# FARIDKH/Multi-agent-RL-for-FJSP

Hardware: AMD Instinct MI355X
Metric: env-steps/sec (all agents) at N parallel envs, 1/2/4/8 MI355X (higher is better)
Workload: dtype int32+f64; 1 GPU; fjsp_step_4096envs; envs_per_gpu=4096, global_envs=4096, num_orders=30, policy=random, steps_per_launch=1024, kernel=k_step_ag<lds,predraw>, bench_step=one rollout batch = 256 env-steps of each of the 4096 envs, env_steps_per_bench_step=1048576, parallelism=env-shard x1 (no data-path collective)

## Files before the change

### multi-agent-rl-for-fjsp_amd/csrc/fjsp_env.h

```cpp
#pragma once
#include <stdint.h>

#include "fjsp_stamps.h"

#ifndef FJSP_DEV
#define FJSP_DEV __device__ __forceinline__
#endif
#ifndef FJSP_HD
#ifdef __HIP__
#define FJSP_HD __host__ __device__ __forceinline__
#else
#define FJSP_HD FJSP_DEV
#endif
#endif

namespace fjsp {

FJSP_DEV float __uint_as_float_fjsp(uint32_t u) { float f; __builtin_memcpy(&f, &u, 4); return f; }
FJSP_DEV uint32_t __float_as_uint_fjsp(float f) { uint32_t u; __builtin_memcpy(&u, &f, 4); return u; }

constexpr int BLOCK = 64;
constexpr int NA = 8;
constexpr int NI32 = 20, NI8 = 12, NF32 = 6, NMASK = 29;
constexpr int MAX_ORDERS = 64;
// ... 637 lines not shown
    return inflight && cs == (uint16_t)step;
}
template <int S, bool AT = false>
FJSP_DEV void pack_run(Env& E, const Tables& T, const Cfg& C, int started, bool due, int* orders_done) {
    constexpr int L = L_PKG + S;
    const int step = E.step();
    const int qfirst = E.p_qfirst(S);
    if (started && E.p_inflight(S) + E.p_queued(S) > C.pkg_cap)
        E.flag(ST_PKG_WAIT | ST_DIVERGED);
    int done = 0;
    while (due) {
        const int s = list_pop<L>(E, T);
        const int code = T.scode[s * T.stride];
        const int o = tc_order(code);
        const uint32_t add = tc_range(code) << 9;
        uint32_t w = (AT ? order_or(&T.orders[o * T.stride], add) : T.orders[o * T.stride]) | add;
        const uint32_t full = (1u << ow_n(w)) - 1u;
        if (!(w & (1u << 18)) && ((w >> 9) & full) == full) {
            w |= 1u << 18;
            *orders_done += 1;
            if (AT) order_or(&T.orders[o * T.stride], 1u << 18);
        }
        if (!AT) T.orders[o * T.stride] = w;
        done += tc_count(code);
        due = E.ll(L) > 0 && E.lh(L) != qfirst && T.scstep[E.lh(L) * T.stride] == PKG_CONT;
    }
    if (done) {
        E.set_p_completed(S, E.p_completed(S) + done);
        E.set_total_packaged(E.total_packaged() + done);
        E.set_p_inflight(S, E.p_inflight(S) - done);
        E.set_p_busy(S, 0);
    }
    if (started) {
        T.scstep[qfirst * T.stride] = (uint16_t)(step + C.ptk_pack);
        const int inflight = E.p_inflight(S) + E.p_queued(S);
        E.w[20 + S] = 3u | ((uint32_t)NIL << 2) | ((uint32_t)(inflight & 0xFF) << 10);
    }
}

template <int S>
FJSP_DEV int pack_complete(Env& E, const Tables& T, bool due, int* orders_done) {
    constexpr int L = L_PKG + S;
    const int qfirst = E.p_qfirst(S);
    int done = 0;
    while (due) {
        const int s = list_pop<L>(E, T);
        const int code = T.scode[s * T.stride];
        const int o = tc_order(code);
        const uint32_t add = tc_range(code) << 9;
        const uint32_t w = order_or(&T.orders[o * T.stride], add) | add;
        const uint32_t full = (1u << ow_n(w)) - 1u;
        if (!(w & (1u << 18)) && ((w >> 9) & full) == full) {
            order_or(&T.orders[o * T.stride], 1u << 18);
            *orders_done += 1;
        }
        done += tc_count(code);
        due = E.ll(L) > 0 && E.lh(L) != qfirst && T.scstep[E.lh(L) * T.stride] == PKG_CONT;
    }
    return done;
}
template <int S>
FJSP_DEV void pack_finish(Env& E, const Tables& T, const Cfg& C, int started, int done) {
    if (started && E.p_inflight(S) + E.p_queued(S) > C.pkg_cap) E.flag(ST_PKG_WAIT | ST_DIVERGED);
    if (done) {
        E.set_p_completed(S, E.p_completed(S) + done);
        E.set_total_packaged(E.total_packaged() + done);
        E.set_p_inflight(S, E.p_inflight(S) - done);
        E.set_p_busy(S, 0);
    }
    if (started) {
        T.scstep[E.p_qfirst(S) * T.stride] = (uint16_t)(E.step() + C.ptk_pack);
        const int inflight = E.p_inflight(S) + E.p_queued(S);
        E.w[20 + S] = 3u | ((uint32_t)NIL << 2) | ((uint32_t)(inflight & 0xFF) << 10);
    }
}

template <int P>
struct PackSlot { static constexpr int value = P; };
template <int P, int NP, class F>
FJSP_DEV void pack_slots(F&& f) {
    if constexpr (P < NP) { f(PackSlot<P>{}); pack_slots<P + 1, NP>(f); }
}
template <int G>
FJSP_DEV uint32_t pack_lane_room(const Env& E, const Cfg& C, int g) {
    uint32_t room = 0;
#pragma unroll
    for (int p = 0; p < 4 / G; p++) room |= (uint32_t)(E.p_inflight(p) < C.pkg_cap) << (p * G + g);
    return room;
}
template <int G>
FJSP_DEV uint32_t pack_lane_step(Env& E, const Tables& T, const Cfg& C, int g, uint32_t a1, uint32_t pend, uint32_t room,
                                 uint32_t* r) {
    constexpr int NP = 4 / G;
    const int step = E.step();
    const uint32_t w1 = E.w[1];
    bool due[NP];
    int done[NP], st[NP], orders_done = 0;
    pack_slots<0, NP>([&](auto p) { due[p.value] = pack_due<p.value>(E, T, step); });
    pack_slots<0, NP>([&](auto p) { done[p.value] = pack_complete<p.value>(E, T, due[p.value], &orders_done); });
    if (pend) {
        const uint32_t cand = (uint32_t)nib(nibs(0, 0x4, 0x3, 0x8, 0, 0), (int)((pend >> 22) & 3u)) & room;
        const int s = __builtin_ffs((int)cand) - 1;
        if (s < 0) E.flag(ST_PROD_LOST);
        else if ((s & (G - 1)) == g) agv_pack_push<NP>(E, T, pend, s / G);
    }
    pack_slots<0, NP>([&](auto p) {
        const int act = (int)((a1 >> (8 * (p.value * G + g))) & 0xFFu);
        st[p.value] = 0;
        r[p.value] = (pack_execute<p.value>(E, act, &st[p.value]) & 0xFFu) | ((uint32_t)act << 8);
    });
    pack_slots<0, NP>([&](auto p) { pack_finish<p.value>(E, T, C, st[p.value], done[p.value]); });
    bool over = false;
#pragma unroll
    for (int p = 0; p < NP; p++) over = over || E.p_queued(p) > 127;
    if (over) E.flag(ST_OBS_OVERFLOW | ST_DIVERGED);
    const uint32_t part = (uint32_t)orders_done | ((uint32_t)(E.total_packaged() - (int)(w1 >> 8)) << 8);
    E.w[1] = w1;
    return part;
}
FJSP_DEV void pack_lane_apply(Env& E, uint32_t sums) { E.w[1] += sums; }
template <int G, class W>
FJSP_DEV void pack_lane_load(Env& E, int g, W&& word) {
    E.w[1] = word(1);
    E.w[24] = 0u; E.w[25] = 0u;
#pragma unroll
    for (int p = 0; p < 4 / G; p++) {
        const int s = p * G + g;
        E.w[7 + L_PKG + p] = word(7 + L_PKG + s);
        E.w[20 + p] = word(20 + s);
        E.w[26 + p] = word(26 + s);
        E.set_p_completed(p, (int)((word(24 + (s >> 1)) >> (16 * (s & 1))) & 0xFFFFu));
    }
}
template <int G>
FJSP_DEV void pack_lane_clear(Env& E) {
    E.w[0] = 0u; E.w[1] = 0u; E.w[2] = 0u;
#pragma unroll
    for (int p = 0; p < 4 / G; p++) {
        E.w[7 + L_PKG + p] = (uint32_t)NIL | ((uint32_t)NIL << 8);
        E.w[20 + p] = (uint32_t)NIL << 2;
        E.w[26 + p] = 0u;
    }
    E.w[24] = 0u; E.w[25] = 0u;
}
template <int G>
FJSP_DEV uint32_t pack_lane_counts(const Env& E, int g, int half) {
    uint32_t v = 0;
#pragma unroll
    for (int p = 0; p < 4 / G; p++) {
        const int s = p * G + g;
        v |= (s >> 1) == half ? (uint32_t)E.p_completed(p) << (16 * (s & 1)) : 0u;
    }
    return v;
}

struct Obs {
    int32_t i32[NI32];
    int8_t i8[NI8];
    float f32[NF32];
    int8_t mask[NMASK];
};
struct ObsSink {
    Obs& o;
    FJSP_DEV void i32(int f, int v) { o.i32[f] = v; }
    FJSP_DEV void i8(int f, int v) { o.i8[f] = (int8_t)v; }
    FJSP_DEV void f32(int f, float v) { o.f32[f] = v; }
    FJSP_DEV void mask(int f, int v) { o.mask[f] = (int8_t)v; }
};
struct MaskBits {
    uint32_t bits[NA] = {0, 0, 0, 0, 0, 0, 0, 0};
    FJSP_DEV void i32(int, int) {}
    FJSP_DEV void i8(int, int) {}
    FJSP_DEV void f32(int, float) {}
    FJSP_DEV void mask(int f, int v) {
        const int a = f < 3 ? 0 : f < 11 ? 1 : 2 + (f - 11) / 3;
        const int off = f < 3 ? 0 : f < 11 ? 3 : 11 + 3 * (a - 2);
        bits[a] |= (uint32_t)(v != 0) << (f - off);
    }
};

template <class Sink>
FJSP_DEV void compute_masks(const Env& E, const Cfg& C, Sink& m) {
    const int co = E.cur_order(), more_orders = E.next_order() < E.norders();
    const int tv = E.tray_valid(), tcnt = E.tray_count();
    const int has_order = co >= 0 || more_orders;
    const int has_tray = tv || E.pool() > 0;
    const int not_full = tv ? (tcnt < C.mask_tray_cap) : 1;
    const int prem = co >= 0 ? (E.cur_idx() < E.cur_n()) : more_orders;
    m.mask(0, 1);
    m.mask(1, has_order && has_tray && not_full && prem);
    m.mask(2, tv && tcnt > 0);
    const int loc = E.loc();
    m.mask(3, 1);
    m.mask(4, loc != LOC_PICKUP);
    m.mask(5, loc != LOC_SMALL);
    m.mask(6, loc != LOC_BIG);
    m.mask(7, loc != LOC_STORAGE);
    m.mask(8, loc != LOC_PACK);
    int pick = 0, drop = 0;
    if (E.carry() == NIL) {
        pick = (loc == LOC_PICKUP && E.ll(L_PREADY) > 0) || (loc == LOC_SMALL && E.ll(L_M0R) > 0) ||
               (loc == LOC_BIG && E.ll(L_M1R) > 0) || (loc == LOC_STORAGE && E.ll(L_STORAGE) > 0);
    } else {
        const int ty = E.carry_type(), np = E.carry_np();
        drop = (loc == LOC_PICKUP && tc_count(E.carry_code()) == 0) ||
               (loc == LOC_SMALL && np && (ty == 1 || ty == 2)) || (loc == LOC_BIG && np && (ty == 3 || ty == 2)) ||
               (loc == LOC_PACK && E.carry_nk() && !np) || (loc == LOC_STORAGE);
    }
    m.mask(9, pick);
    m.mask(10, drop);
    m.mask(11, 1); m.mask(12, E.ll(L_M0Q) > 0 && !E.m_busy(0)); m.mask(13, !E.m_busy(0) && E.m_cur(0) != NIL);
    m.mask(14, 1); m.mask(15, E.ll(L_M1Q) > 0 && !E.m_busy(1)); m.mask(16, !E.m_busy(1) && E.m_cur(1) != NIL);
#pragma unroll
    for (int s = 0; s < 4; s++) {
        const int busy = E.p_busy(s);
        m.mask(17 + 3 * s, 1);
        m.mask(18 + 3 * s, E.p_queued(s) > 0 && !busy && E.p_inflight(s) < C.pkg_cap);
        m.mask(19 + 3 * s, !busy && E.p_hascur(s));
    }
}

FJSP_DEV float pack_progress(const Cfg& C, int n) {
    if (__builtin_expect(n >= RPROG_N, 0)) return (float)((1.0 / (double)n) * 100.0);
    return (float)C.lut[RPROG + n];
}

FJSP_DEV int obs_i8_checked(Env& E, int v) {
    if (v > 127) E.flag(ST_OBS_OVERFLOW | ST_DIVERGED);
    return (int)(int8_t)v;
}

template <class Sink>
FJSP_DEV void observe(Env& E, const Cfg& C, Sink& o) {
    int osz = 0, rem = 0, npt = 0, npc = 0;
    const int co = E.cur_order();
    if (co >= 0) {
        osz = E.cur_n(); rem = osz - E.cur_idx();
        if (rem > 0) { npt = E.cur_type(); npc = E.cur_color(); }
    }
    int tt = 0, tcol = 0, tcnt = 0;
    if (E.tray_valid()) {
        tcnt = E.tray_count();
        if (tcnt > 0 && E.tray_order() == co) {
            tt = E.cur_type(); tcol = E.cur_color();
        }
    }
    o.i32(0, osz); o.i32(1, rem); o.i32(2, npt); o.i32(3, npc);
    o.i32(4, tt); o.i32(5, tcol); o.i32(6, tcnt);
    const int c = E.carry() != NIL, loc = E.loc();
    o.i32(7, loc_row(loc)); o.i32(8, loc_col(loc));
    o.i32(9, c);
    o.i32(10, c ? tc_count(E.carry_code()) : 0);
    o.i32(11, c ? E.carry_type() : 0);
    o.i32(12, c ? E.carry_np() : 0);
    o.i32(13, c ? E.carry_nk() : 0);
    o.i32(14, E.ll(L_PREADY));
    o.i32(15, E.m_busy(0)); o.i32(16, E.m_busy(1));
    o.i32(17, E.ll(L_M0R)); o.i32(18, E.ll(L_M1R));
    o.i32(19, E.ll(L_STORAGE));
    o.i8(0, E.m_busy(0)); o.i8(1, obs_i8_checked(E, E.ll(L_M0Q)));
    o.i8(2, E.m_busy(1)); o.i8(3, obs_i8_checked(E, E.ll(L_M1Q)));
    o.f32(0, E.m_prog(0) ? 1.0f : 0.0f);
    o.f32(1, E.m_prog(1) ? 1.0f : 0.0f);
#pragma unroll
    for (int s = 0; s < 4; s++) {
        o.i8(4 + 2 * s, E.p_busy(s));
        o.i8(5 + 2 * s, obs_i8_checked(E, E.p_queued(s)));
        o.f32(2 + s, pack_progress(C, E.p_startn(s)));
    }
    compute_masks(E, C, o);
}

FJSP_DEV void station_i8(const Env& E, int8_t* v) {
    v[0] = (int8_t)E.m_busy(0); v[1] = (int8_t)E.ll(L_M0Q);
    v[2] = (int8_t)E.m_busy(1); v[3] = (int8_t)E.ll(L_M1Q);
#pragma unroll
    for (int s = 0; s < 4; s++) {
        v[4 + 2 * s] = (int8_t)E.p_busy(s);
        v[5 + 2 * s] = (int8_t)E.p_queued(s);
    }
}

FJSP_DEV uint32_t held_word(bool holds, int code) {
    return holds ? (1u << 13) | (tc_count(code) != 0 ? (uint32_t)code : 0u) : 0u;
}
FJSP_DEV void held_words(const Env& E, uint32_t v[3]) {
    v[0] = held_word(E.carry() != NIL, E.carry_code()) | ((uint32_t)E.loc() << 16);
#pragma unroll
    for (int m = 0; m < 2; m++) v[1 + m] = held_word(E.m_cur(m) != NIL, E.m_code(m)) | ((uint32_t)E.m_busy(m) << 14);
}

FJSP_DEV void pack_words(const Env& E, uint32_t v[4]) {
#pragma unroll
    for (int s = 0; s < 4; s++)
        v[s] = ((uint32_t)E.ll(L_PKG + s) & 0xFFu) | (((uint32_t)(E.p_queued(s) + E.p_inflight(s)) & 0xFFFu) << 8) |
               (((uint32_t)E.p_completed(s) & 0xFFFu) << 20);
}

FJSP_DEV int machine_available(const Env& E, int m) {
    return !E.m_busy(m) && E.ll(m == 0 ? L_M0Q : L_M1Q) < 3;
}
FJSP_DEV void heuristic_actions(const Env& E, const Tables& T, int* act) {
    const int has_orders = E.next_order() < E.norders() || E.cur_order() >= 0;
    act[0] = has_orders ? 1 : 0;
    const int loc = E.loc();
    int a = 0;
// ... 132 lines not shown
```

### multi-agent-rl-for-fjsp_amd/csrc/fjsp_hip.hip

```cpp
#include <hip/hip_runtime.h>
#include <stdint.h>
#include <stdio.h>
#include <stdlib.h>
#include <string.h>
#include <chrono>
#include <string>
#include <type_traits>

#include "fjsp_env.h"
#include "fjsp_orders.h"
#include "fjsp_select.h"
#include "fjsp_stamps.h"
#include "fjsp_stepdev.h"
#include "../../include/fjsp.h"

using namespace fjsp;

namespace {

FJSP_DIAG(__device__ unsigned long long g_stamps[8];
          __device__ unsigned long long g_pgstamps[4];
          __device__ unsigned long long g_emitstamps[4];
          __device__ unsigned long long g_agstamps[64];)

// ... 812 lines not shown
        E.st_t0 = __builtin_amdgcn_s_memtime();
        )
        int epi = 0;
        for (int k = 0; k <= K; k++) {
            if (k < K && valid) {
                int act[NA];
                if (pre) {
                    const uint32_t a0 = s_act[k & 1][0][lane], a1 = s_act[k & 1][1][lane];
#pragma unroll
                    for (int a = 0; a < 4; a++) { act[a] = (a0 >> (8 * a)) & 0xFF; act[4 + a] = (a1 >> (8 * a)) & 0xFF; }
                } else {
                    synth_actions(seed, gid0 + (uint32_t)e, step0 + (uint32_t)k, mode, E, T, C, act);
                }
                FJSP_STAMP(E, 0);
                uint32_t res[NA];
                const int nc0 = E.ncompleted(), tp0 = E.total_packaged();
                (void)env_advance<true>(E, T, C, act, nullptr, res);
                flag_obs_overflow(E);
                uint32_t v[SNAP_N];
                int j = 0;
#pragma unroll
                for (int i = 0; i < NSTATE; i++)
                    if ((SNAP_WORDS >> i) & 1u) v[j++] = E.w[i];
#pragma unroll
                for (int a = 0; a < NA; a++) v[SNAP_RES + a] = res[a] | ((uint32_t)act[a] << 8);
                v[SNAP_GSTAT] = (uint32_t)(E.ncompleted() - nc0) | ((uint32_t)(E.total_packaged() - tp0) << 16);
#pragma unroll
                for (int i = SNAP_GSTAT + 1; i < SNAP_N; i++) v[i] = 0u;
                snap_put(snap[k & 1], lane, v);
                const int nord = E.norders();
                const int all_done = E.ncompleted() == nord && nord > 0 && E.next_order() == nord;
                const int truncated = E.step() >= C.max_steps;
                FJSP_STAMP(E, 3);
                E.set_step(E.step() + 1);
                if (autoreset && (all_done || truncated)) {
                    if constexpr (PG) {
                        const uint32_t pr = s_mb[2][k & 1][lane];
                        if ((pr & 1u) && ((pr >> 1) & 0xFFu) == (uint32_t)epi && (int)((pr >> 9) & 0x7Fu) == nord)
                            env_reset_predrawn(E, T, C, nord, s_mb[3][k & 1][lane], s_nxt + lane);
                        else
                            E = env_reset_cold(E, T, C, S, e, nord, false);
                        epi = (epi + 1) & 0xFF;
                    } else {
                        E = env_reset_cold(E, T, C, S, e, nord);
                    }
                }
                if constexpr (PG) {
                    s_mb[0][(k + 1) & 1][lane] = (uint32_t)epi | ((uint32_t)E.norders() << 8);
                    s_mb[1][(k + 1) & 1][lane] = E.w[3];
                }
                FJSP_STAMP(E, 6);
            }
            __syncthreads();
        }
        if (valid) {
            if constexpr (LDS) tables_copy_out(S, T, e, E.norders(), E.slot_next());
            env_store(E, S.words, S.n, e);
        }
        FJSP_DIAG(
        if (lane == 0)
            for (int i = 0; i < 8; i++) atomicAdd((unsigned long long*)&g_stamps[i], (unsigned long long)E.st_acc[i]);
        )
    } else if (PG && wave == 1 + NEMIT) {
        predraw_wave<CR, PB>(S, K, lane, e, valid, (size_t)blockIdx.x * BLOCK, s_mb, s_cp, s_nxt);
    } else {
        const int part = wave - 1;
        const PipeArgs* pa = kargs_flat<PipeArgs>();
        const Cfg C = cfg_at(pa, s_lut);
        const fjsp_out out = out_at(pa->out);
        const uint64_t seed = pa->seed;
        const uint32_t gid0 = pa->gid0, step0 = pa->step0;
        FJSP_DIAG(
        uint64_t em_busy = 0;
        )
        for (int k = 0; k <= K; k++) {
            FJSP_DIAG(
            const uint64_t et0 = __builtin_amdgcn_s_memtime();
            )
            if (part == 0 && pre && k + 1 < K) {
                int act_next[NA];
                synth_uniform(seed, gid0 + (uint32_t)e, step0 + (uint32_t)(k + 1), act_next);
                s_act[(k + 1) & 1][0][lane] = pack_actions(act_next, 0);
                s_act[(k + 1) & 1][1][lane] = pack_actions(act_next, 4);
            }
            const bool have = k > 0 && valid;
            const uint32_t t = (uint32_t)(k - 1);
            uint32_t v[SNAP_N];
            Env E;
            if (have) {
                snap_get(snap[(k - 1) & 1], lane, v);
                int j = 0;
#pragma unroll
                for (int i = 0; i < NSTATE; i++) E.w[i] = ((SNAP_WORDS >> i) & 1u) ? v[j++] : 0u;
            }
            const StoreSink sink{out.obs_i32, out.obs_i8, out.obs_f32, out.masks, t, n, ue};
            if (part == 0 && have && out.rewards) {
                const uint32_t gs = v[SNAP_GSTAT];
                const double g8 = global_reward8(C, (int)(gs & 0xFFFFu), (int)(gs >> 16));
#pragma unroll
                for (int a = 0; a < NA; a++) {
                    const uint32_t r = v[SNAP_RES + a];
                    st32(out.rewards, (t * NA + (uint32_t)a) * n + ue,
                         g8 + C.lut[reward_index(a, r & 0xFFFF00FFu, (int)((r >> 8) & 0xFu))]);
                }
            }
            if (have) {
                if (part == 0) {
                    PartSink<NEMIT == 1 ? -1 : 0> ps{sink};
                    observe(E, C, ps);
                }
                if (part == NEMIT - 1) {
                    if (NEMIT == 2) {
                        PartSink<1> ps{sink};
                        observe(E, C, ps);
                    }
                    const int nord = E.norders();
                    const int all_done = E.ncompleted() == nord && nord > 0 && E.next_order() == nord;
                    const int truncated = E.step() >= C.max_steps;
                    if (out.term) st32(out.term, t * n + ue, (uint8_t)all_done);
                    if (out.trunc) st32(out.trunc, t * n + ue, (uint8_t)truncated);
                    if (out.status) st32(out.status, t * n + ue, E.status());
                }
            }
            FJSP_DIAG(
            em_busy += __builtin_amdgcn_s_memtime() - et0;
            )
            __syncthreads();
        }
        FJSP_DIAG(
        if (lane == 0 && part < 2) {
            atomicAdd(&g_emitstamps[2 * part], (unsigned long long)em_busy);
            atomicAdd(&g_emitstamps[2 * part + 1], (unsigned long long)(K + 1));
        }
        )
    }
}

constexpr int AG_AM = 0, AG_P = 1, AG_E1 = 2, AG_E2 = 3, AG_E0 = 5, AG_E3 = 7;
static_assert(AG_WAVES == 8, "one wave per role (AG_WAVES: fjsp_select.h)");
constexpr uint32_t K_WORDS = (1u << 1) | (0xFu << 13) | (0x3FFu << 20);
template <bool AMK, int E0ST, int E1ST>
struct AgSplitOf {
    static constexpr bool AM_K = AMK;
    static constexpr uint32_t E0ST_BITS = ((1u << (3 * E0ST)) - 1u) << 11, E1ST_BITS = ((1u << (3 * E1ST)) - 1u) << (11 + 3 * E0ST);
    static constexpr uint32_t MASKS_E0 = 0x7u | E0ST_BITS, MASKS_E1 = E1ST_BITS, MASKS_E2 = (0x3u << 9) | (0x3Fu << 3),
                              MASKS_E3 = (0x3FFFFu << 11) & ~(E0ST_BITS | E1ST_BITS);
    static_assert(E0ST + E1ST <= 6, "two machines and four packaging stations");
    static_assert((MASKS_E0 | MASKS_E1 | MASKS_E2 | MASKS_E3) == (1u << NMASK) - 1u &&
                  __builtin_popcount(MASKS_E0) + __builtin_popcount(MASKS_E1) + __builtin_popcount(MASKS_E2) +
                  __builtin_popcount(MASKS_E3) == NMASK, "mask split");
};
template <int G> struct AgSplit : AgSplitOf<false, 2, 4> {};
template <> struct AgSplit<4> : AgSplitOf<true, 2, 4> {};
enum : int { SA_W0 = 0, SA_ST, SA_W4, SA_W5, SA_W6, SA_L0, SA_M0 = SA_L0 + 6, SA_M1, SA_R01, SA_R23,
             SK_W1 = 16 };
template <int G>
struct SnapK {
    static constexpr int ST = G == 1 ? 25 : 17, GS = G == 1 ? 26 : 18, P0 = G == 1 ? 17 : 20, N0 = G == 1 ? 21 : 24,
                         R45 = G == 1 ? 27 : 28, R67 = R45 + 1;
    static_assert(G == 1 || (SK_W1 % 4 == 0 && GS < SK_W1 + 4 && P0 % 4 == 0 && N0 % 4 == 0 && R45 % 4 == 0),
                  "K's snapshot words");
    static_assert(R67 < 32, "snapshot slot");
};
static_assert(SA_R23 < 16, "snapshot slot");
enum : int { RS_NO = 0, RS_W4, RS_W5, RS_R0 = RS_W5 + 8, RS_R1, RS_ST, RS_PEND = 15, RS_N };
static_assert(RS_N <= 16, "s_res slot");
enum : int { P1_W0 = 0, P1_W4, P1_W5, P1_W6, P1_W7, P1_W8, P1_PEND, P1_N };
__device__ __forceinline__ void q_get(const uint4* q, int ng, uint32_t* v) {
#pragma unroll
    for (int g = 0; g < ng; g++) {
        const uint4 x = q[g * BLOCK];
        v[4 * g] = x.x; v[4 * g + 1] = x.y; v[4 * g + 2] = x.z; v[4 * g + 3] = x.w;
    }
}
__device__ __forceinline__ void q_put(uint4* q, int ng, const uint32_t* v) {
#pragma unroll
    for (int g = 0; g < ng; g++) q[g * BLOCK] = make_uint4(v[4 * g], v[4 * g + 1], v[4 * g + 2], v[4 * g + 3]);
}

template <int G>
__device__ __forceinline__ uint32_t lanes_or(uint32_t x) {
    if constexpr (G >= 4) x |= (uint32_t)__shfl_xor((int)x, BLOCK / 4);
    if constexpr (G >= 2) x |= (uint32_t)__shfl_xor((int)x, BLOCK / 2);
    return x;
}
template <int G>
__device__ __forceinline__ uint32_t lanes_sum(uint32_t x) {
    if constexpr (G >= 4) x += (uint32_t)__shfl_xor((int)x, BLOCK / 4);
    if constexpr (G >= 2) x += (uint32_t)__shfl_xor((int)x, BLOCK / 2);
    return x;
}

__device__ __forceinline__ void snap_put4(PipeSnap& sp, int q0, int lane, const uint32_t* v) {
#pragma unroll
    for (int g = 0; g < 4; g++) sp.q[q0 + g][lane] = make_uint4(v[4 * g], v[4 * g + 1], v[4 * g + 2], v[4 * g + 3]);
}

__device__ __forceinline__ bool ag_fresh(int k, bool valid, const uint4 (*s_p1)[2][BLOCK], const uint32_t (*s_kpost)[BLOCK],
                                         int lane, const Cfg& C, int autoreset) {
    if (k == 0) return true;
    if (!valid) return false;
    const uint32_t w0a = s_p1[(k - 1) & 1][0][lane].x;
    const int nord = (int)((w0a >> 16) & 0xFFu);
    const int all_done = (int)(s_kpost[(k - 1) & 1][lane] & 0xFFu) == nord && nord > 0 && (int)(w0a >> 24) == nord;
    return autoreset && (all_done || (int)(w0a & 0xFFFFu) >= C.max_steps);
}

__device__ __forceinline__ void ag_pin(AgvPre& a) {
#define AG_PIN(x) asm volatile("" : "+v"(x))
#pragma unroll
    for (int i = 0; i < 6; i++) AG_PIN(a.m[i]);
    AG_PIN(a.lw_own); AG_PIN(a.delta); AG_PIN(a.keep); AG_PIN(a.orb); AG_PIN(a.edge_len); AG_PIN(a.edge_val);
    AG_PIN(a.force); AG_PIN(a.thr); AG_PIN(a.w6[0]); AG_PIN(a.w6[1]); AG_PIN(a.r[0]);
    AG_PIN(a.r[1]); AG_PIN(a.pend); AG_PIN(a.pool_add); AG_PIN(a.st); AG_PIN(a.carry);
#undef AG_PIN
}

template <int part, int G>
__device__ __forceinline__ void ag_emit(const uint32_t* v, uint32_t t, uint32_t n, uint32_t ue, const Cfg& C,
                                        const fjsp_out& out) {
    using SK = SnapK<G>;
    Env E;
#pragma unroll
    for (int i = 0; i < NSTATE; i++) E.w[i] = 0u;
    E.w[0] = v[SA_W0]; E.w[2] = v[SA_ST] | v[SK::ST]; E.w[4] = v[SA_W4]; E.w[5] = v[SA_W5];
    E.w[6] = v[SA_W6];
#pragma unroll
    for (int l = 0; l < 6; l++) E.w[7 + l] = v[SA_L0 + l];
    E.w[17] = v[SA_M0]; E.w[18] = v[SA_M1];
    E.w[1] = v[SK_W1];
#pragma unroll
    for (int s = 0; s < 4; s++) { E.w[20 + s] = v[SK::P0 + s]; E.w[26 + s] = v[SK::N0 + s]; }
    const StoreSink sink{out.obs_i32, out.obs_i8, out.obs_f32, out.masks, t, n, ue};
    if (part == 0) {
        if (out.rewards) {
            const uint32_t gs = v[SK::GS];
            const double g8 = global_reward8(C, (int)(gs & 0xFFFFu), (int)(gs >> 16));
            const uint32_t rw[4] = {v[SA_R01], v[SA_R23], v[SK::R45], v[SK::R67]};
#pragma unroll
            for (int a = 0; a < NA; a++) {
                const uint32_t r = (rw[a >> 1] >> (16 * (a & 1))) & 0xFFFFu;
                st32(out.rewards, (t * NA + (uint32_t)a) * n + ue,
                     g8 + C.lut[reward_index(a, r & 0xFFu, (int)((r >> 8) & 0xFu))]);
            }
        }
        FieldSink<0u, 0u, 0u, AgSplit<G>::MASKS_E0> ps{sink};
        observe(E, C, ps);
    } else if (part == 1) {
        FieldSink<(1u << NI32) - 1u, 0u, (1u << NF32) - 1u, AgSplit<G>::MASKS_E1> ps{sink};
        observe(E, C, ps);
    } else if (part == 3) {
        FieldSink<0u, 0u, 0u, AgSplit<G>::MASKS_E3> ps{sink};
        observe(E, C, ps);
    } else {
        FieldSink<0u, (1u << NI8) - 1u, 0u, AgSplit<G>::MASKS_E2> ps{sink};
        observe(E, C, ps);
        const int nord = E.norders();
        const int all_done = E.ncompleted() == nord && nord > 0 && E.next_order() == nord;
        const int truncated = E.step() >= C.max_steps;
        if (out.term) st32(out.term, t * n + ue, (uint8_t)all_done);
        if (out.trunc) st32(out.trunc, t * n + ue, (uint8_t)truncated);
        if (out.status) st32(out.status, t * n + ue, E.status());
    }
}


template <int EPW, bool STALL = false>
__global__ void __launch_bounds__(AG_WAVES * BLOCK) __attribute__((amdgpu_waves_per_eu(1, 2)))
k_step_ag(DevState S, Cfg Ck, int K, uint64_t seed, uint32_t gid0, uint32_t step0, int autoreset, fjsp_out out) {
    static_assert(EPW == 64 || EPW == 32 || EPW == 16, "envs per workgroup");
    constexpr int AG_K = AgSplit<BLOCK / EPW>::AM_K ? 4 : 6, AG_PD = AgSplit<BLOCK / EPW>::AM_K ? 6 : 4;
    FJSP_DIAG(
    const uint64_t t_entry = __builtin_amdgcn_s_memtime();
    )
    constexpr int CR = PG_CR, PB = AG_PB;
    __shared__ uint32_t s_orders[MAX_ORDERS * BLOCK];
    __shared__ uint32_t s_nxt[MAX_ORDERS * BLOCK];
    __shared__ uint32_t s_mb[4][2][BLOCK];
    __shared__ uint4 s_cp[1][3][BLOCK];
    __shared__ uint16_t s_code[MAX_SLOTS * BLOCK];
    __shared__ uint8_t s_next[MAX_SLOTS * BLOCK];
    __shared__ uint16_t s_cstep[MAX_SLOTS * BLOCK];
    __shared__ PipeSnap snap[2];
    __shared__ uint32_t s_act[4][2][BLOCK];
    __shared__ uint4 s_p1[2][2][BLOCK];
    __shared__ uint4 s_p2[BLOCK];
    __shared__ uint4 s_res[2][4][BLOCK];
    __shared__ uint32_t s_kpost[3][BLOCK];
    __shared__ uint32_t s_flag1;
    __shared__ uint32_t s_uflag;
    __shared__ uint32_t s_abort;
    __shared__ uint32_t s_cap;
    __shared__ uint4 s_pk[BLOCK];
    __shared__ uint2 s_pkr[BLOCK];
    __shared__ double s_lut[RLUT_SIZE];
    for (int i = threadIdx.x; i < RLUT_SIZE; i += AG_WAVES * BLOCK) s_lut[i] = Ck.lut[i];
    const int wave = __builtin_amdgcn_readfirstlane(threadIdx.x / BLOCK);
    const int lane = threadIdx.x % BLOCK;
    const int blk = xcd_block((int)blockIdx.x, (int)gridDim.x);
    const int e = blk * EPW + lane;
    const bool valid = lane < EPW && e < S.n;
    const uint32_t n = (uint32_t)S.n, ue = (uint32_t)e;
    const Tables TL{s_orders + lane, s_code + lane, s_next + lane, s_cstep + lane, BLOCK};
    FJSP_DIAG(uint64_t ag_busy = 0, ag_wait = 0;
              uint64_t amt[6] = {0, 0, 0, 0, 0, 0};
              uint64_t ag_last = 0;)
    if (wave == AG_P) {
        for (int j = 0; j < 3 && j < K; j++) {
            int act[NA];
            synth_uniform(seed, gid0 + (uint32_t)e, step0 + (uint32_t)j, act);
            s_act[j][0][lane] = pack_actions(act, 0);
            s_act[j][1][lane] = pack_actions(act, 4);
        }
    }
    if (threadIdx.x == 0) { s_flag1 = 0; s_uflag = 0; s_abort = 0; s_cap = aux_words(S)[AUX_SPIN_CAP]; }
    auto ag_spin = [&](uint32_t* flag, uint32_t v) __attribute__((always_inline)) {
        spin_until(flag, v, &s_abort, &s_cap);
    };
    auto ag_spin2 = [&](uint32_t* f1, uint32_t* f2, uint32_t v) __attribute__((always_inline)) {
        const uint32_t a = __hip_atomic_load(f1, __ATOMIC_RELAXED, __HIP_MEMORY_SCOPE_WORKGROUP);
        const uint32_t b = __hip_atomic_load(f2, __ATOMIC_RELAXED, __HIP_MEMORY_SCOPE_WORKGROUP);
        if (__builtin_amdgcn_readfirstlane((a ^ v) | (b ^ v)) == 0u) {
            __builtin_amdgcn_fence(__ATOMIC_ACQUIRE, "workgroup");
            return;
        }
        spin_until(f1, v, &s_abort, &s_cap);
        spin_until(f2, v, &s_abort, &s_cap);
    };
    if (valid) {
        const uint32_t w0 = S.words[e], w5 = S.words[5 * n + e], pg = S.words[(size_t)PGW * n + e];
        uint32_t ov[MAX_ORDERS / AG_WAVES], pv[MAX_ORDERS / AG_WAVES];
#pragma unroll
        for (int j = 0; j < MAX_ORDERS / AG_WAVES; j++) {
            const size_t o = (size_t)(wave + AG_WAVES * j);
            ov[j] = S.orders[o * n + e];
            pv[j] = S.nxt[o * n + e];
        }
        uint32_t cv[8], xv[8], tv[8];
#pragma unroll
        for (int j = 0; j < 4; j++) {
            const size_t q = (size_t)(wave + AG_WAVES * j);
            cv[j] = S.scode[q * n + e];
            xv[j] = S.snext[q * n + e];
            tv[j] = S.scstep[q * n + e];
        }
        const uint32_t nslots = w5 >> 24;
        const uint32_t no = (w0 >> 16) & 0xFFu, npd = (pg & 1u) ? (pg >> 24) & 0x7Fu : 0u;
#pragma unroll
        for (int j = 0; j < MAX_ORDERS / AG_WAVES; j++) {
            const uint32_t o = (uint32_t)(wave + AG_WAVES * j);
            if (o < no) TL.orders[o * BLOCK] = ov[j];
            if (o < npd) s_nxt[o * BLOCK + lane] = pv[j];
        }
#pragma unroll
        for (int j = 0; j < 4; j++) {
            const uint32_t q = (uint32_t)(wave + AG_WAVES * j);
            if (q < nslots) {
                TL.scode[q * BLOCK] = (uint16_t)cv[j];
                TL.snext[q * BLOCK] = (uint8_t)xv[j];
                TL.scstep[q * BLOCK] = (uint16_t)tv[j];
            }
        }
        for (uint32_t q0 = (uint32_t)wave + 4 * AG_WAVES; q0 < nslots; q0 += 8 * AG_WAVES) {
#pragma unroll
            for (int j = 0; j < 8; j++) {
                const uint32_t q = q0 + (uint32_t)(AG_WAVES * j);
                cv[j] = q < nslots ? S.scode[(size_t)q * n + e] : 0u;
                xv[j] = q < nslots ? S.snext[(size_t)q * n + e] : 0u;
                tv[j] = q < nslots ? S.scstep[(size_t)q * n + e] : 0u;
            }
#pragma unroll
            for (int j = 0; j < 8; j++) {
                const uint32_t q = q0 + (uint32_t)(AG_WAVES * j);
                if (q < nslots) {
                    TL.scode[q * BLOCK] = (uint16_t)cv[j];
                    TL.snext[q * BLOCK] = (uint8_t)xv[j];
                    TL.scstep[q * BLOCK] = (uint16_t)tv[j];
                }
            }
        }
        if (wave == AG_AM) {
            s_mb[0][0][lane] = no << 8;
            s_mb[1][0][lane] = S.words[3 * n + e];
        }
        if (wave == AG_PD) {
            s_mb[2][0][lane] = (pg & 1u) ? 1u | (npd << 9) : 0u;
            s_mb[3][0][lane] = (pg & 1u) ? ((pg >> 1) & 0x3FFu) | (((pg >> 11) & 0x3FFu) << 16) | (((pg >> 21) & 1u) << 31) : 0u;
        }
    }
    __syncthreads();
    FJSP_DIAG(
    if (threadIdx.x == 0) atomicAdd(&g_agstamps[56], (unsigned long long)(__builtin_amdgcn_s_memtime() - t_entry));
    )
    if constexpr (STALL) {
        if (wave == AG_AM && blockIdx.x == 0) stall_for_test(S);
    }
    if (wave == AG_AM) {
        Cfg C = cfg_at(ag_args(), s_lut);
        asm volatile("" : "+v"(C.max_steps), "+v"(C.tray_cap), "+v"(C.storage_cap), "+v"(C.pool0), "+v"(C.ptk_small),
                          "+v"(C.ptk_big));
        __builtin_amdgcn_s_setprio(3);
        Env E;
        if (valid) env_load(E, S.words, S.n, e);
        int epi = 0;
        bool fresh = true, trunc_prev = false;
        FJSP_DIAG(
        const uint64_t loop_t0 = __builtin_amdgcn_s_memtime();
        )
        for (int k = 0; k <= K; k++) {
            AG_T0();
            AG_MARK(0);
            int pl0 = 0, pl1 = 0, pn0 = NIL, pn1 = NIL;
            if (valid && k < K) {
                pl0 = E.ll(L_M0Q);
                pl1 = E.ll(L_M1Q);
                if (pl0 >= 2) pn0 = TL.snext[E.lh(L_M0Q) * BLOCK];
                if (pl1 >= 2) pn1 = TL.snext[E.lh(L_M1Q) * BLOCK];
            }
            uint32_t kc = 0, a0 = 0, a1 = 0, rs[16];
            if (valid) {
                kc = s_kpost[(k - 1) & 1][lane];
                if (k < K) {
                    a0 = s_act[k & 3][0][lane];
                    a1 = s_act[k & 3][1][lane];
                    q_get(&s_res[k & 1][0][lane], 4, rs);
                }
            }
            if (valid) {
                if (k > 0) {
                    const int nord = E.norders();
                    const int all_done = (int)(kc & 0xFFu) == nord && nord > 0 && E.next_order() == nord;
                    if (autoreset && (all_done || trunc_prev)) {
                        fresh = true;
                        const uint32_t pr = s_mb[2][k & 1][lane];
                        if ((pr & 1u) && ((pr >> 1) & 0xFFu) == (uint32_t)epi && (int)((pr >> 9) & 0x7Fu) == nord)
                            env_reset_predrawn(E, TL, C, nord, s_mb[3][k & 1][lane], s_nxt + lane);
                        else
                            E = env_reset_cold(E, TL, C, S, e, nord, false);
                        epi = (epi + 1) & 0xFF;
                    }
                }
            }
            AG_MARK(1);
            if (k < K && valid) {
                int act[NA];
#pragma unroll
                for (int a = 0; a < 4; a++) { act[a] = (a0 >> (8 * a)) & 0xFF; act[4 + a] = (a1 >> (8 * a)) & 0xFF; }
                uint32_t r0, r1, pend = 0;
                if (!fresh) {
                    E.w[0] = (E.w[0] & 0x00FFFFFFu) | (rs[RS_NO] << 24);
                    E.w[4] = rs[RS_W4];
#pragma unroll
                    for (int i = 0; i < 8; i++) E.w[5 + i] = rs[RS_W5 + i];
                    r0 = rs[RS_R0];
                    r1 = rs[RS_R1];
                    E.w[2] |= rs[RS_ST];
                } else {
                    r0 = (pickup_execute(E, TL, C, act[0]) & 0xFFu) | ((uint32_t)act[0] << 8);
                    int mv = 0;
                    r1 = (agv_execute<true>(E, TL, C, act[1], &mv, &pend) & 0xFFu) | ((uint32_t)act[1] << 8);
                    if (mv) E.set_loc(mv);
                }
                AG_MARK(2);
                int s0 = -1, s1 = -1;
                const int nk0 = fresh ? -1 : pl0 >= 2 ? pn0 : E.lt(L_M0Q);
                const int nk1 = fresh ? -1 : pl1 >= 2 ? pn1 : E.lt(L_M1Q);
                const uint32_t r2 = (machine_execute<0>(E, TL, act[2], &s0, nk0) & 0xFFu) | ((uint32_t)act[2] << 8);
                const uint32_t r3 = (machine_execute<1>(E, TL, act[3], &s1, nk1) & 0xFFu) | ((uint32_t)act[3] << 8);
                AG_MARK(3);
                {
                    const uint32_t p1[8] = {E.w[0], E.w[4], E.w[5], E.w[6], E.w[7], E.w[8], pend, 0u};
                    q_put(&s_p1[k & 1][0][lane], 2, p1);
                    s_p2[lane] = make_uint4(E.w[9], E.w[10], E.w[11], E.w[12]);
                }
                __hip_atomic_store(&s_flag1, (uint32_t)(k + 1), __ATOMIC_RELEASE, __HIP_MEMORY_SCOPE_WORKGROUP);
                AG_ACC(ag_wait);
                AG_MARK(4);
                machines_run<true>(E, TL, C, s0, s1);
                AG_MARK(5);
                if (E.ll(L_M0Q) > 127 || E.ll(L_M1Q) > 127) E.flag(ST_OBS_OVERFLOW | ST_DIVERGED);
                const uint32_t v[16] = {E.w[0], E.w[2], E.w[4], E.w[5], E.w[6], E.w[7], E.w[8], E.w[9], E.w[10],
                                        E.w[11], E.w[12], E.w[17], E.w[18], r0 | (r1 << 16), r2 | (r3 << 16), 0u};
                snap_put4(snap[k & 1], 0, lane, v);
                trunc_prev = E.step() >= C.max_steps;
                E.set_step(E.step() + 1);
                fresh = false;
            }
            if (valid) {
                s_mb[0][(k + 1) & 1][lane] = (uint32_t)epi | ((uint32_t)E.norders() << 8);
                s_mb[1][(k + 1) & 1][lane] = E.w[3];
            }
            AG_ACC(ag_busy);
            AG_BARRIER();
        }
        FJSP_DIAG(
        if (lane == 0) atomicAdd(&g_agstamps[24], (unsigned long long)(__builtin_amdgcn_s_memtime() - loop_t0));
        )
        if (valid) {
            s_act[0][0][lane] = (uint32_t)E.norders();
            s_act[0][1][lane] = (uint32_t)E.slot_next();
            E.w[2] |= s_kpost[2][lane];
            if (s_abort) E.w[2] |= ST_SPIN_TIMEOUT | ST_DIVERGED;
#pragma unroll
            for (int i = 0; i < NSTATE; i++)
                if (!((K_WORDS >> i) & 1u)) S.words[i * n + e] = E.w[i];
        }
    } else if (wave == AG_K) {
        constexpr int G = BLOCK / EPW, NP = 4 / G;
        const Cfg C = cfg_at(ag_args(), s_lut);
        __builtin_amdgcn_s_setprio(2);
        const int g = lane / EPW, el = lane % EPW;
        const int ek = blk * EPW + el;
        const bool kvalid = ek < S.n;
        const Tables TK{s_orders + el, s_code + el, s_next + el, s_cstep + el, BLOCK};
        Env E;
#pragma unroll
        for (int i = 0; i < NSTATE; i++) E.w[i] = 0u;
        if (kvalid) {
            pack_lane_load<G>(E, g, [&](int i) { return S.words[(size_t)i * n + ek]; });
            E.w[0] = S.words[ek] & 0xFFFFu;
        }
        bool trunc_prev = false;
        for (int k = 0; k <= K; k++) {
            AG_T0();
            bool fresh = k == 0;
            if (kvalid && k > 0) {
                const uint32_t w0a = s_p1[(k - 1) & 1][0][el].x;
                const int nord = (int)((w0a >> 16) & 0xFFu);
                const int all_done = E.ncompleted() == nord && nord > 0 && (int)(w0a >> 24) == nord;
                if (autoreset && (all_done || trunc_prev)) {
                    fresh = true;
                    pack_lane_clear<G>(E);
                }
            }
            if (k < K) {
                uint32_t pend = 0;
                if (k == 0) {
                    AG_SPIN_T0();
                    ag_spin(&s_flag1, 1u);
                    AG_SPIN_ACC();
                    if (kvalid) pend = s_p1[0][1][el].z;
                } else if (kvalid && !fresh) {
                    pend = s_res[k & 1][RS_PEND / 4][el].w;
                }
                if (kvalid) {
                    const int step = E.step();
                    const uint32_t a1 = s_act[k & 3][1][el];
                    if constexpr (G == 1) {
                        const int tp0 = E.total_packaged();
                        int done[4], orders_done = 0;
// ... 1339 lines not shown
```

Baseline: 4.294 billion env-steps/s.

## Split AM wave's two machines across lane groups when multiple envs share a wave

When each wave holds more than one lane group (BLOCK/EPW > 1), the AM wave now runs machine 0 and machine 1 for an env on separate lane groups instead of serially in one lane. Shared env state is broadcast with shuffles after fresh resets, each group writes its own snapshot words, and a new SnapA layout packs the second machine's words plus extra status bits. The aim is to shorten the AM wave's critical path per step by using idle lanes. In exchange it adds shuffles, atomic order updates and more complex snapshot packing, which may introduce divergence.

```diff
diff --git a/multi-agent-rl-for-fjsp_amd/csrc/fjsp_env.h b/multi-agent-rl-for-fjsp_amd/csrc/fjsp_env.h
--- a/multi-agent-rl-for-fjsp_amd/csrc/fjsp_env.h
+++ b/multi-agent-rl-for-fjsp_amd/csrc/fjsp_env.h
@@ -813,6 +813,45 @@
         v |= (s >> 1) == half ? (uint32_t)E.p_completed(p) << (16 * (s & 1)) : 0u;
     }
     return v;
+}
+
+template <class W>
+FJSP_DEV void mach_lane_load(Env& E, int g, W&& word) {
+    E.w[7 + L_M0Q] = word(7 + L_M0Q + 2 * g);
+    E.w[7 + L_M0R] = word(7 + L_M0R + 2 * g);
+    E.w[17] = word(17 + g);
+    E.w[19] = (word(19) >> (16 * g)) & 0xFFFFu;
+}
+FJSP_DEV void mach_lane_clear(Env& E) {
+    E.w[0] = 0u; E.w[2] = 0u;
+    E.w[7 + L_M0Q] = (uint32_t)NIL | ((uint32_t)NIL << 8);
+    E.w[7 + L_M0R] = (uint32_t)NIL | ((uint32_t)NIL << 8);
+    E.w[17] = (uint32_t)NIL << 1;
+    E.w[19] = 0u;
+}
+template <bool AT = false>
+FJSP_DEV void mach_lane_run(Env& E, const Tables& T, int ptk, int s0) {
+    const int step = E.step();
+    const bool due0 = E.m_busy(0) && E.m_next(0) == step;
+    const int c0 = E.m_code(0);
+    const int o0 = tc_order(c0);
+    const int g0 = T.scode[(s0 >= 0 ? s0 : 0) * T.stride];
+    const uint32_t b0 = 1u << (tc_start(c0) + E.m_k(0));
+    if (due0) {
+        if constexpr (AT) order_or(&T.orders[o0 * T.stride], b0);
+        else T.orders[o0 * T.stride] |= b0;
+        const int k = E.m_k(0);
+        E.set_m_k(0, k + 1);
+        if (k + 1 >= tc_count(c0)) { E.set_m_busy(0, 0); E.set_m_prog(0, 1); }
+        else E.set_m_next(0, step + ptk);
+    }
+    if (s0 >= 0) {
+        if (E.m_cur(0) != NIL) E.flag(ST_OVERWRITE);
+        const int busy = tc_count(g0) > 0;
+        E.set_m_grant(0, s0, g0, busy);
+        if (busy) E.set_m_next(0, step + ptk);
+        else E.set_m_prog(0, 1);
+    }
 }
 
 struct Obs {
diff --git a/multi-agent-rl-for-fjsp_amd/csrc/fjsp_hip.hip b/multi-agent-rl-for-fjsp_amd/csrc/fjsp_hip.hip
--- a/multi-agent-rl-for-fjsp_amd/csrc/fjsp_hip.hip
+++ b/multi-agent-rl-for-fjsp_amd/csrc/fjsp_hip.hip
@@ -988,8 +988,13 @@
 };
 template <int G> struct AgSplit : AgSplitOf<false, 2, 4> {};
 template <> struct AgSplit<4> : AgSplitOf<true, 2, 4> {};
-enum : int { SA_W0 = 0, SA_ST, SA_W4, SA_W5, SA_W6, SA_L0, SA_M0 = SA_L0 + 6, SA_M1, SA_R01, SA_R23,
-             SK_W1 = 16 };
+enum : int { SA_W0 = 0, SA_ST, SA_W4, SA_W5, SA_W6, SK_W1 = 16 };
+template <int G>
+struct SnapA {
+    static constexpr int L(int l) { return G == 1 ? 5 + l : l < 2 ? 5 + l : l < 4 ? 6 + l : 8 + l; }
+    static constexpr int M0 = G == 1 ? 11 : 10, M1 = G == 1 ? 12 : 14, R01 = G == 1 ? 13 : 7, R23 = G == 1 ? 14 : 11, X = 15;
+    static_assert(G == 1 || (L(0) == 5 && L(1) == 6 && L(2) == 8 && L(3) == 9 && L(4) == 12 && L(5) == 13), "AM's snapshot words");
+};
 template <int G>
 struct SnapK {
     static constexpr int ST = G == 1 ? 25 : 17, GS = G == 1 ? 26 : 18, P0 = G == 1 ? 17 : 20, N0 = G == 1 ? 21 : 24,
@@ -998,7 +1003,6 @@
                   "K's snapshot words");
     static_assert(R67 < 32, "snapshot slot");
 };
-static_assert(SA_R23 < 16, "snapshot slot");
 enum : int { RS_NO = 0, RS_W4, RS_W5, RS_R0 = RS_W5 + 8, RS_R1, RS_ST, RS_PEND = 15, RS_N };
 static_assert(RS_N <= 16, "s_res slot");
 enum : int { P1_W0 = 0, P1_W4, P1_W5, P1_W6, P1_W7, P1_W8, P1_PEND, P1_N };
@@ -1059,11 +1063,13 @@
     Env E;
 #pragma unroll
     for (int i = 0; i < NSTATE; i++) E.w[i] = 0u;
+    using SA = SnapA<G>;
     E.w[0] = v[SA_W0]; E.w[2] = v[SA_ST] | v[SK::ST]; E.w[4] = v[SA_W4]; E.w[5] = v[SA_W5];
+    if constexpr (G > 1) E.w[2] |= v[SA::X] >> 16;
     E.w[6] = v[SA_W6];
 #pragma unroll
-    for (int l = 0; l < 6; l++) E.w[7 + l] = v[SA_L0 + l];
-    E.w[17] = v[SA_M0]; E.w[18] = v[SA_M1];
+    for (int l = 0; l < 6; l++) E.w[7 + l] = v[SA::L(l)];
+    E.w[17] = v[SA::M0]; E.w[18] = v[SA::M1];
     E.w[1] = v[SK_W1];
 #pragma unroll
     for (int s = 0; s < 4; s++) { E.w[20 + s] = v[SK::P0 + s]; E.w[26 + s] = v[SK::N0 + s]; }
@@ -1072,7 +1078,7 @@
         if (out.rewards) {
             const uint32_t gs = v[SK::GS];
             const double g8 = global_reward8(C, (int)(gs & 0xFFFFu), (int)(gs >> 16));
-            const uint32_t rw[4] = {v[SA_R01], v[SA_R23], v[SK::R45], v[SK::R67]};
+            const uint32_t rw[4] = {v[SA::R01], G > 1 ? v[SA::R23] | (v[SA::X] << 16) : v[SA::R23], v[SK::R45], v[SK::R67]};
 #pragma unroll
             for (int a = 0; a < NA; a++) {
                 const uint32_t r = (rw[a >> 1] >> (16 * (a & 1))) & 0xFFFFu;
@@ -1231,7 +1237,156 @@
     if constexpr (STALL) {
         if (wave == AG_AM && blockIdx.x == 0) stall_for_test(S);
     }
-    if (wave == AG_AM) {
+    if (BLOCK / EPW > 1 && wave == AG_AM) {
+        if constexpr (BLOCK / EPW > 1) {
+        using SA = SnapA<BLOCK / EPW>;
+        Cfg C = cfg_at(ag_args(), s_lut);
+        asm volatile("" : "+v"(C.max_steps), "+v"(C.tray_cap), "+v"(C.storage_cap), "+v"(C.pool0), "+v"(C.ptk_small),
+                          "+v"(C.ptk_big));
+        __builtin_amdgcn_s_setprio(3);
+        const int g = lane / EPW, el = lane % EPW;
+        const int em = blk * EPW + el;
+        const bool mval = g < 2 && em < S.n, v1 = mval && g == 1;
+        const Tables TM{s_orders + el, s_code + el, s_next + el, s_cstep + el, BLOCK};
+        const int ptk = g ? C.ptk_big : C.ptk_small;
+        Env E;
+#pragma unroll
+        for (int i = 0; i < NSTATE; i++) E.w[i] = 0u;
+        if (valid) env_load(E, S.words, S.n, e);
+        if (v1) {
+            mach_lane_load(E, 1, [&](int i) { return S.words[(size_t)i * n + em]; });
+            E.w[0] = S.words[em];
+        }
+        int epi = 0;
+        bool fresh = true, trunc_prev = false;
+        FJSP_DIAG(
+        const uint64_t loop_t0 = __builtin_amdgcn_s_memtime();
+        )
+        for (int k = 0; k <= K; k++) {
+            AG_T0();
+            AG_MARK(0);
+            int pl = 0, pn = NIL;
+            if (mval && k < K) {
+                pl = E.ll(L_M0Q);
+                if (pl >= 2) pn = TM.snext[E.lh(L_M0Q) * BLOCK];
+            }
+            uint32_t kc = 0, a0 = 0, rs[16];
+            if (mval) {
+                kc = s_kpost[(k - 1) & 1][el];
+                if (k < K) {
+                    a0 = s_act[k & 3][0][el];
+                    q_get(&s_res[k & 1][0][el], 4, rs);
+                }
+            }
+            if (mval && k > 0) {
+                const int nord = E.norders();
+                const int all_done = (int)(kc & 0xFFu) == nord && nord > 0 && E.next_order() == nord;
+                if (autoreset && (all_done || trunc_prev)) {
+                    fresh = true;
+                    if (g == 0) {
+                        const uint32_t pr = s_mb[2][k & 1][lane];
+                        if ((pr & 1u) && ((pr >> 1) & 0xFFu) == (uint32_t)epi && (int)((pr >> 9) & 0x7Fu) == nord)
+                            env_reset_predrawn(E, TL, C, nord, s_mb[3][k & 1][lane], s_nxt + lane);
+                        else
+                            E = env_reset_cold(E, TL, C, S, e, nord, false);
+                        epi = (epi + 1) & 0xFF;
+                    } else {
+                        mach_lane_clear(E);
+                        E.set_norders(nord);
+                    }
+                }
+            }
+            AG_MARK(1);
+            if (k < K) {
+                uint32_t r0 = 0, r1 = 0, pend = 0;
+                if (mval && !fresh) {
+                    E.w[0] = (E.w[0] & 0x00FFFFFFu) | (rs[RS_NO] << 24);
+                    E.w[4] = rs[RS_W4];
+#pragma unroll
+                    for (int i = 0; i < 8; i++) E.w[5 + i] = rs[RS_W5 + i];
+                    E.w[7 + L_M0Q] = g ? rs[RS_W5 + 2 + L_M1Q] : rs[RS_W5 + 2 + L_M0Q];
+                    E.w[7 + L_M0R] = g ? rs[RS_W5 + 2 + L_M1R] : rs[RS_W5 + 2 + L_M0R];
+                    r0 = rs[RS_R0];
+                    r1 = rs[RS_R1];
+                    E.w[2] |= g ? 0u : rs[RS_ST];
+                }
+                if (__ballot(mval && fresh) != 0) {
+                    if (valid && fresh) {
+                        const int act0 = (int)(a0 & 0xFFu), act1 = (int)((a0 >> 8) & 0xFFu);
+                        r0 = (pickup_execute(E, TL, C, act0) & 0xFFu) | ((uint32_t)act0 << 8);
+                        int mv = 0;
+                        r1 = (agv_execute<true>(E, TL, C, act1, &mv, &pend) & 0xFFu) | ((uint32_t)act1 << 8);
+                        if (mv) E.set_loc(mv);
+                    }
+                    const uint32_t h0 = (uint32_t)__shfl((int)E.w[0], el);
+                    const uint32_t hq = (uint32_t)__shfl((int)E.w[7 + L_M1Q], el), hr = (uint32_t)__shfl((int)E.w[7 + L_M1R], el);
+                    if (v1 && fresh) {
+                        E.w[0] = h0;
+                        E.w[7 + L_M0Q] = hq;
+                        E.w[7 + L_M0R] = hr;
+                    }
+                }
+                AG_MARK(2);
+                if (mval) {
+                    const int actm = (int)((a0 >> (16 + 8 * g)) & 0xFFu);
+                    int s0 = -1;
+                    const int nk = fresh ? -1 : pl >= 2 ? pn : E.lt(L_M0Q);
+                    const uint32_t rm2 = (machine_execute<0>(E, TM, actm, &s0, nk) & 0xFFu) | ((uint32_t)actm << 8);
+                    AG_MARK(3);
+                    if (g == 0) {
+                        const uint32_t p1[8] = {E.w[0], E.w[4], E.w[5], E.w[6], E.w[7], E.w[8], pend, 0u};
+                        q_put(&s_p1[k & 1][0][lane], 2, p1);
+                    }
+                    reinterpret_cast<uint2*>(&s_p2[el])[g] = make_uint2(E.w[7 + L_M0Q], E.w[7 + L_M0R]);
+                    __hip_atomic_store(&s_flag1, (uint32_t)(k + 1), __ATOMIC_RELEASE, __HIP_MEMORY_SCOPE_WORKGROUP);
+                    AG_ACC(ag_wait);
+                    AG_MARK(4);
+                    mach_lane_run<true>(E, TM, ptk, s0);
+                    AG_MARK(5);
+                    if (E.ll(L_M0Q) > 127) E.flag(ST_OBS_OVERFLOW | ST_DIVERGED);
+                    if (g == 0) {
+                        const uint32_t v[12] = {E.w[0], E.w[2], E.w[4], E.w[5], E.w[6], E.w[7], E.w[8], r0 | (r1 << 16),
+                                                E.w[9], E.w[10], E.w[17], rm2};
+                        static_assert(SA::R01 == 7 && SA::L(2) == 8 && SA::M0 == 10 && SA::R23 == 11, "group 0's snapshot words");
+#pragma unroll
+                        for (int q = 0; q < 3; q++) snap[k & 1].q[q][lane] = make_uint4(v[4 * q], v[4 * q + 1], v[4 * q + 2], v[4 * q + 3]);
+                    } else {
+                        static_assert(SA::L(4) == 12 && SA::M1 == 14 && SA::X == 15, "group 1's snapshot words");
+                        snap[k & 1].q[3][el] = make_uint4(E.w[7 + L_M0Q], E.w[7 + L_M0R], E.w[17], rm2 | (E.w[2] << 16));
+                    }
+                    trunc_prev = E.step() >= C.max_steps;
+                    E.set_step(E.step() + 1);
+                    fresh = false;
+                }
+            }
+            if (valid) {
+                s_mb[0][(k + 1) & 1][lane] = (uint32_t)epi | ((uint32_t)E.norders() << 8);
+                s_mb[1][(k + 1) & 1][lane] = E.w[3];
+            }
+            AG_ACC(ag_busy);
+            AG_BARRIER();
+        }
+        FJSP_DIAG(
+        if (lane == 0) atomicAdd(&g_agstamps[24], (unsigned long long)(__builtin_amdgcn_s_memtime() - loop_t0));
+        )
+        const uint32_t n1 = (uint32_t)__shfl((int)E.w[19], EPW + el), st1 = (uint32_t)__shfl((int)E.w[2], EPW + el);
+        if (v1) {
+            S.words[(size_t)(7 + L_M1Q) * n + em] = E.w[7 + L_M0Q];
+            S.words[(size_t)(7 + L_M1R) * n + em] = E.w[7 + L_M0R];
+            S.words[(size_t)18 * n + em] = E.w[17];
+        }
+        if (valid) {
+            s_act[0][0][lane] = (uint32_t)E.norders();
+            s_act[0][1][lane] = (uint32_t)E.slot_next();
+            E.w[2] |= s_kpost[2][lane] | st1;
+            E.w[19] = (E.w[19] & 0xFFFFu) | (n1 << 16);
+            if (s_abort) E.w[2] |= ST_SPIN_TIMEOUT | ST_DIVERGED;
+#pragma unroll
+            for (int i = 0; i < NSTATE; i++)
+                if (!((K_WORDS >> i) & 1u) && i != 7 + L_M1Q && i != 7 + L_M1R && i != 18) S.words[i * n + e] = E.w[i];
+        }
+        }
+    } else if (wave == AG_AM) {
         Cfg C = cfg_at(ag_args(), s_lut);
         asm volatile("" : "+v"(C.max_steps), "+v"(C.tray_cap), "+v"(C.storage_cap), "+v"(C.pool0), "+v"(C.ptk_small),
                           "+v"(C.ptk_big));
```

After: 4.409 billion env-steps/s (median of 6 runs). 2.7% higher.
